# ebiggers/libdeflate

Measured on AMD Instinct MI355X. Metric: compress+decompress MB/s, 64 KiB chunks level 6, higher is better.
Workload: dtype u8

## Files before the change

libdeflate_amd/csrc/deflate_blockend.h:

```cpp

static __device__ u32 block_scan(lds_t *L, u32 v, u32 *total)
{
	const u32 lane = threadIdx.x & 63, wave = threadIdx.x >> 6;
	u32 incl = wave_scan_incl(v);

	if (lane == 63)
		L->scan[0][wave] = incl;
	__syncthreads();
	const u32 sw = lane < NWAVES ? L->scan[0][lane] : 0;
	const u32 iw = wave_scan_incl(sw);
	const u32 base = bcast_lane(iw - sw, wave);
	__syncthreads();
	*total = bcast_lane(iw, NWAVES - 1);
	return base + incl - v;
}

static __device__ u32 block_scan1(lds_t *L, u32 v, u32 *total,
				  u32 *tog)
{
	const u32 lane = threadIdx.x & 63, wave = threadIdx.x >> 6;
	u32 incl = wave_scan_incl(v);
	u32 *sc = L->scan[*tog];

	*tog ^= 1;
// ... 46 lines not shown

static __device__ __forceinline__ u32 *stg_of(lds_t *L)
{
	return (u32 *)L->nxtA;
}

static __device__ __forceinline__ void
stg_put(lds_t *L, const struct outstate *os, u64 bitpos, u64 code,
	u32 nbits)
{
	if (!nbits)
		return;
	u64 rel = bitpos - 8 * os->sg;
	u32 w = (u32)(rel >> 5), s = (u32)rel & 31;
	u32 *stg = stg_of(L);
	u64 lo = code << s;
	atomicOr((u32 *)&stg[w], (u32)lo);
	if (s + nbits > 32)
		atomicOr((u32 *)&stg[w + 1], (u32)(lo >> 32));
	if (s + nbits > 64)
		atomicOr((u32 *)&stg[w + 2], (u32)(code >> (64 - s)));
}

static __device__ __forceinline__ void
stg_flush(lds_t *L, struct outstate *os, bool final)
{
	u32 *stg = stg_of(L);
	u8 *stgb = (u8 *)stg;
	const u32 tid = threadIdx.x;
	u64 done_bytes = final ? (os->bits + 7) / 8 : os->bits / 8;
	u64 rel_end = done_bytes - os->sg;
	s64 first = -(s64)os->sg;
	u32 start = first > 0 ? (u32)first : 0;
	u32 units = final ? (u32)((rel_end + 15) / 16) : (u32)(rel_end / 16);

	__syncthreads();
	for (u32 u = tid; u < units; u += NT) {
		u32 b0 = u * 16, b1 = b0 + 16;
		u8 *g = os->out + (s64)(os->sg + b0);
		if (b0 >= start && b1 <= rel_end) {
			*(uint4 *)g = *(const uint4 *)(stgb + b0);
		} else {
			for (u32 b = b0 < start ? start : b0; b < b1 && b < rel_end; b++)
				g[b - b0] = stgb[b];
		}
	}
	u32 keep_from = units * 16;
	u32 total_words = (u32)((os->bits - 8 * os->sg + 31) / 32) + 1;
	u32 keep_words = final ? 0 : total_words - keep_from / 4;
	u32 v = 0;
	if (tid < keep_words && keep_from / 4 + tid < STG_WORDS + 8)
		v = stg[keep_from / 4 + tid];
	__syncthreads();
	for (u32 i = tid; i < STG_WORDS + 8; i += NT)
		stg[i] = 0;
	if (tid < keep_words)
		stg[tid] = v;
	os->sg += keep_from;
}

static __device__ __forceinline__ void stg_restore(lds_t *L)
{
	u32 *stg = stg_of(L);

	__syncthreads();
	for (u32 i = threadIdx.x; i < STG_WORDS + 8; i += NT)
		stg[i] = i < 6 ? L->carry[i] : 0;
	__syncthreads();
}

static __device__ __forceinline__ void stg_save(lds_t *L, struct outstate *os)
{
	stg_flush(L, os, false);
	if (threadIdx.x < 6)
		L->carry[threadIdx.x] = stg_of(L)[threadIdx.x];
	__syncthreads();
}

static __device__ __forceinline__ void
put_container_header(lds_t *L, struct outstate *os, int format, int level,
		     const u8 *__restrict__ dict_pre, u32 hdr_bytes, u32 tid)
{
	if (tid == 0) {
		if (format == LDA_FMT_BGZF) {
			stg_put(L, os, 0, 0x04088B1Full, 32);
			stg_put(L, os, 32, 0, 32);
			stg_put(L, os, 64, 0xFFu << 8, 16);
			stg_put(L, os, 80, 0x0243420006ull, 48);
		} else if (format == LDA_FMT_GZIP) {
			u32 xfl = level < 2 ? 4 : level >= 8 ? 2 : 0;
			stg_put(L, os, 0, 0x00088B1Full, 32);
			stg_put(L, os, 32, 0, 32);
			stg_put(L, os, 64, xfl | (0xFFu << 8), 16);
		} else {
			u32 fl = level < 2 ? 0 : level < 6 ? 1 :
				 level < 8 ? 2 : 3;
			u32 h = (0x78u << 8) | (fl << 6);
			if (dict_pre) {
				h |= 0x20;
				h += (31 - h % 31) % 31;
				stg_put(L, os, 16, __builtin_bswap32(((const u32 *)dict_pre)[1]), 32);
			} else {
				h |= 31 - (h % 31);
			}
			stg_put(L, os, 0, ((h & 0xFF) << 8) | (h >> 8), 16);
		}
	}
	os->bits = 8 * hdr_bytes;
}

static __device__ __forceinline__ bool
block_emit(lds_t *L, struct outstate *os, const u32 *__restrict__ tokg, u32 nseq,
	   const u8 *__restrict__ inp, u32 bstart, u32 blen, u32 is_final,
	   bool stored_only, u32 ftr_bytes, u32 *tog, u32 tid, u32 lane, u32 wave)
{
	PROF_DECL;
	PROF_START();
	u32 btype = 0;
	if (!stored_only) {
		if (tid == 0)
			L->freq[256]++;
		__syncthreads();
		{
			u32 *keys = L->M;
			u32 *usedv = L->M + 320;
			u16 *sortedO = (u16 *)(L->M + 324);
			if (tid < 2)
				usedv[tid] = 0;
			__syncthreads();
			for (u32 vt = tid; vt < 320; vt += NT) {
				const u32 f = L->freq[vt];
				if (f) {
					if (vt < 288)
						keys[atomicAdd(&usedv[0], 1u)] = (f << 9) | vt;
					else
						keys[288 + atomicAdd(&usedv[1], 1u)] =
							(f << 9) | (vt - 288);
				}
			}
			__syncthreads();
			{
				const u32 m1 = usedv[0], m2 = usedv[1];
				for (u32 i = tid; i < m1 + m2; i += NT) {
					const bool lit = i < m1;
					const u32 lo = lit ? 0 : 288, m = lit ? m1 : m2;
					const u32 key = keys[lit ? i : 288 + i - m1];
					u32 r = 0;
					for (u32 q = 0; q < m; q++)
						r += keys[lo + q] < key;
					if (lit)
						L->sorted[r] = (u16)(key & 511);
					else
						sortedO[r] = (u16)(key & 511);
				}
			}
			__syncthreads();
			PROF_MARK(10);
			if (wave == 0)
				make_code(L->freq, 288, 15, L->lens, L->codes,
					  L->sorted, HUFF_LITLEN(L),
					  usedv[0], true, lane);
			else if (wave == 1)
// ... 141 lines not shown
			u32 xb = tid == 16 ? 2 : tid == 17 ? 3 : tid == 18 ? 7 : 0;
			dyn += L->pre_freq[tid] * (L->pre_lens[tid] + xb);
		}
		u32 dyn_tot, stat_tot;
		(void)block_scan(L, dyn, &dyn_tot);
		(void)block_scan(L, stat, &stat_tot);
		static const u8 perm[19] = { 16, 17, 18, 0, 8, 7, 9, 6, 10,
					     5, 11, 4, 12, 3, 13, 2, 14,
					     1, 15 };
		u32 nexp = 19;
		while (nexp > 4 && L->pre_lens[perm[nexp - 1]] == 0)
			nexp--;
		u32 cost_dyn = 3 + 5 + 5 + 4 + 3 * nexp + dyn_tot;
		u32 cost_stat = 3 + stat_tot;
		u32 pieces = blen ? (blen + 65534) / 65535 : 1;
		u32 pad = (u32)((0 - (os->bits + 3)) & 7);
		u64 cost_stored = 3 + pad + 32 + 8ull * blen +
				  (u64)(pieces - 1) * 40;
		u64 best = cost_stored;
		btype = 0;
		if (cost_stat < best) {
			best = cost_stat;
			btype = 1;
		}
		if (cost_dyn < best) {
			best = cost_dyn;
			btype = 2;
		}
		if ((os->bits + best + 7) / 8 + ftr_bytes > os->avail)
			return false;
		L->vars[V_TMP3] = nexp;
	} else {
		u32 pieces = blen ? (blen + 65534) / 65535 : 1;
		u64 cost = (u64)pieces * 40 + 8ull * blen;
		if ((os->bits + cost + 7) / 8 + ftr_bytes > os->avail)
			return false;
	}

	PROF_MARK(7);
	stg_restore(L);
	if (btype == 0) {
		u32 done = 0;
		do {
			u32 piece = blen - done > 65535 ? 65535 : blen - done;
			u32 fin = (is_final && done + piece == blen) ? 1 : 0;
			u32 pad = (u32)((0 - (os->bits + 3)) & 7);
			if (tid == 0) {
				stg_put(L, os, os->bits, fin, 3);
				u64 b = os->bits + 3 + pad;
				stg_put(L, os, b, piece | ((u64)(piece ^ 0xFFFF) << 16), 32);
			}
			os->bits += 3 + pad + 32;
			__syncthreads();
			for (u32 w0 = 0; w0 < piece; w0 += 2048) {
				u32 cnt = piece - w0 < 2048 ? piece - w0 : 2048;
				stg_flush(L, os, false);
				__syncthreads();
				for (u32 j = tid; j < cnt; j += NT) {
					u32 pos = bstart + done + w0 + j;
					stg_put(L, os, os->bits + 8ull * j, inp[pos], 8);
				}
				os->bits += 8ull * cnt;
				__syncthreads();
			}
			done += piece;
		} while (done < blen);
		stg_flush(L, os, false);
	} else {
		if (btype == 1) {
			__syncthreads();
			for (u32 s = tid; s < 320; s += NT)
				L->lens[s] = s < 144 ? 8 : s < 256 ? 9 :
					     s < 280 ? 7 : s < 288 ? 8 : 5;
			__syncthreads();
			if (tid == 0) {
				u32 nc[16] = { 0 }, bl[16] = { 0 };
				for (u32 s = 0; s < 288; s++)
					bl[L->lens[s]]++;
				u32 code = 0;
				for (u32 d = 1; d < 16; d++) {
					code = (code + bl[d - 1]) << 1;
					nc[d] = code;
				}
				for (u32 s = 0; s < 288; s++) {
					u32 l = L->lens[s];
					L->codes[s] = (u16)(__brev(nc[l]++) >> (32 - l));
				}
				for (u32 s = 0; s < 32; s++)
					L->codes[288 + s] = (u16)(__brev(s) >> 27);
			}
			__syncthreads();
		}
		{
			u64 hcode[VPT];
			u32 hbits[VPT], hsum = 0;
			const u32 nexp = btype == 2 ? L->vars[V_TMP3] : 0;
			const u32 ni = btype == 2 ? L->vars[V_NPRE] : 0;
#pragma unroll
			for (u32 j = 0; j < VPT; j++) {
				const u32 vt = tid * VPT + j;
				hcode[j] = 0;
				hbits[j] = 0;
				if (vt == 0) {
					hcode[j] = is_final | (btype << 1);
					hbits[j] = 3;
					if (btype == 2) {
						u32 nlit = L->vars[V_TMP1], noff = L->vars[V_TMP2];
						hcode[j] |= (u64)((nlit - 257) | ((noff - 1) << 5) |
								  ((nexp - 4) << 10)) << 3;
						hbits[j] = 17;
					}
				} else if (vt <= nexp) {
					static const u8 perm2[19] = { 16, 17, 18, 0, 8, 7,
						9, 6, 10, 5, 11, 4, 12, 3, 13, 2, 14, 1, 15 };
					hcode[j] = L->pre_lens[perm2[vt - 1]];
					hbits[j] = 3;
				} else if (vt <= nexp + ni) {
					u32 it = L->pre_items[vt - nexp - 1];
					u32 sym = it & 31, ex = it >> 5;
					u32 l = L->pre_lens[sym];
					u32 xb = sym == 16 ? 2 : sym == 17 ? 3 :
						 sym == 18 ? 7 : 0;
					hcode[j] = L->pre_codes[sym] | ((u64)ex << l);
					hbits[j] = l + xb;
				}
				hsum += hbits[j];
			}
			u32 htot;
			u32 hoff = block_scan(L, hsum, &htot);
#pragma unroll
			for (u32 j = 0; j < VPT; j++) {
				stg_put(L, os, os->bits + hoff, hcode[j], hbits[j]);
				hoff += hbits[j];
			}
			os->bits += htot;
		}
		stg_flush(L, os, false);

		PROF_MARK(9);
		__builtin_amdgcn_fence(__ATOMIC_ACQUIRE, "workgroup");
		u32 tok_nxt = tid < nseq ? tokg[tid] : 0;
		for (u32 b0 = 0; b0 < nseq; b0 += NT) {
			u64 code = 0;
			u32 nb = 0;
			const u32 tok = tok_nxt;
			if (b0 + NT + tid < nseq)
				tok_nxt = tokg[b0 + NT + tid];
			if (b0 + tid < nseq) {
				if (tok & TOK_MATCH) {
					const u32 len = (tok & 0xFF) + 3, dist = ((tok >> 8) & 0x7FFF) + 1;
					u32 sl, xb, xv, ds, dxb, dxv;
					length_code(len, &sl, &xb, &xv);
					dist_code(dist, &ds, &dxb, &dxv);
					u32 ll = L->lens[257 + sl];
					u32 dl = L->lens[288 + ds];
					u64 v = L->codes[257 + sl];
					u32 sh = ll;
					v |= (u64)xv << sh;
					sh += xb;
					v |= (u64)L->codes[288 + ds] << sh;
					sh += dl;
					v |= (u64)dxv << sh;
					sh += dxb;
					code = v;
					nb = sh;
				} else {
					code = L->codes[tok];
					nb = L->lens[tok];
				}
			}
			u32 tot;
			u32 off = block_scan1(L, nb, &tot, tog);
			stg_put(L, os, os->bits + off, code, nb);
			os->bits += tot;
			if (os->bits - 8 * os->sg + 48 * NT + 64 > 32 * STG_WORDS)
				stg_flush(L, os, false);
		}
		stg_flush(L, os, false);
		__syncthreads();
		if (tid == 0)
			stg_put(L, os, os->bits, L->codes[256], L->lens[256]);
		os->bits += L->lens[256];
		__syncthreads();
	}

	stg_save(L, os);
	PROF_MARK(8);
	return true;
}

static __device__ __forceinline__ void
finish_stream(lds_t *L, struct outstate *os, bool overflow, bool seg_last,
	      int format, u32 ftr_bytes, const u32 *__restrict__ sums, u64 c, u32 n,
	      u64 *__restrict__ out_nbytes, u32 tid)
{
	__syncthreads();
	if (!overflow && !seg_last &&
	    (os->bits + 3 + 7) / 8 + 4 > os->avail)
		overflow = true;
	if (!overflow) {
		stg_restore(L);
		if (!seg_last) {
			u64 fb = 8 * ((os->bits + 3 + 7) / 8);
			if (tid == 0)
				stg_put(L, os, fb, 0xFFFF0000ull, 32);
			os->bits = fb + 32;
			__syncthreads();
		}
		if (ftr_bytes) {
			u32 sum = sums ? sums[c] : 0;
			u64 fb = 8 * ((os->bits + 7) / 8);
			if (tid == 0) {
				if (format != LDA_FMT_ZLIB) {
					stg_put(L, os, fb, sum, 32);
					stg_put(L, os, fb + 32, n, 32);
				} else {
					stg_put(L, os, fb, __builtin_bswap32(sum), 32);
				}
			}
			os->bits = fb + 8 * ftr_bytes;
			__syncthreads();
		}
		stg_flush(L, os, true);
		const u32 size = (u32)((os->bits + 7) / 8);
		if (tid == 0)
			out_nbytes[c] = size;
		if (format == LDA_FMT_BGZF) {
			asm volatile("s_waitcnt vmcnt(0)" ::: "memory");
			__syncthreads();
			if (tid == 0) {
				const u16 bsize = (u16)(size - 1);
// ... 9 lines not shown
```

libdeflate_amd/csrc/deflate_entropy.hip:

```cpp
#include <stddef.h>
#include "device_common.h"
#include "kernels.h"

#define LDA_ENTROPY 1
#define NT LDA_DEFLATE_ENTROPY_THREADS
#define VPT (1024 / NT)
#define NWAVES (NT / 64)
#ifndef ENTROPY_WGS
#define ENTROPY_WGS 4
#endif
static_assert(NT == 256, "ENTROPY_WGS waves per EU are ENTROPY_WGS workgroups per CU");
#define TOK_MATCH 0x80000000u
#define STG_WORDS 1020

struct deflate_lds {
	u32 M[1776];
	u32 freq[320];
	u8 lens[320];
	u16 codes[320];
	u16 sorted[288];
	u32 hw[288];
	u16 pre_items[320 + 8];
	u32 pre_freq[19];
	u8 pre_lens[20];
	u16 pre_codes[20];
	u32 nxtA[STG_WORDS + 8] __attribute__((aligned(16)));
	u32 scan[2][NWAVES + 1];
	u32 carry[6];
	u32 vars[4];
};
static_assert(sizeof(struct deflate_lds) * ENTROPY_WGS <= 163840, "ENTROPY_WGS workgroups per CU");

#ifdef __HIP_DEVICE_COMPILE__
#define AS3 __attribute__((address_space(3)))
#else
#define AS3
#endif
typedef AS3 struct deflate_lds lds_t;

enum { V_TMP1 = 0, V_TMP2, V_TMP3, V_NPRE, V_COUNT };
static_assert(V_COUNT <= sizeof(((struct deflate_lds *)0)->vars) / sizeof(u32), "vars[] holds them all");

#include "deflate_huffman.h"
#include "deflate_blockend.h"

extern "C" __global__ void __launch_bounds__(NT, ENTROPY_WGS)
lda_deflate_entropy_kernel(u64 n_chunks, int format, int level,
			   const u8 *__restrict__ in_base, const u64 *__restrict__ in_offsets,
			   const u64 *__restrict__ in_nbytes, u8 *__restrict__ out_base,
			   const u64 *__restrict__ out_offsets,
			   const u64 *__restrict__ out_avail_arr, u64 *__restrict__ out_nbytes,
			   const u32 *__restrict__ sums, const u32 *__restrict__ seg_info,
			   const u32 *__restrict__ tok_buf, const u32 *__restrict__ blk_buf,
			   u32 tok_stride, u32 blk_stride)
{
	extern __shared__ __attribute__((aligned(16))) u8 lds_raw[];
	lds_t *L = (lds_t *)(uintptr_t)0;
	const u32 tid = threadIdx.x, lane = tid & 63, wave = tid >> 6;
	if ((u32)(uintptr_t)(__attribute__((address_space(3))) u8 *)lds_raw != 0)
		__builtin_trap();
	const u64 c = blockIdx.x;
	if (c >= n_chunks)
		return;
	const u32 nb = blk_buf[c];
	if (nb == LDA_BLK_FUSED)
		return;
	const u32 *__restrict__ desc = blk_buf + LDA_BLK_HDR_WORDS(n_chunks) +
				       c * blk_stride * LDA_BLK_WORDS;
	const u32 *__restrict__ tokg = tok_buf + c * tok_stride;
	const u8 *__restrict__ inp = in_base + in_offsets[c];
	const u32 n = (u32)in_nbytes[c];
	const bool seg_last = seg_info ? seg_info[c] >> 31 : true;
	const u32 hdr_bytes = format == LDA_FMT_GZIP ? 10 : format == LDA_FMT_BGZF ? 18 :
			      format == LDA_FMT_ZLIB ? 2 : 0;
	const u32 ftr_bytes = format == LDA_FMT_GZIP || format == LDA_FMT_BGZF ? 8 :
			      format == LDA_FMT_ZLIB ? 4 : 0;
	bool overflow = nb == LDA_BLK_OVERFLOW;
	struct outstate os;
	os.out = out_base + out_offsets[c];
	os.avail = out_avail_arr[c];
	if (format == LDA_FMT_BGZF && os.avail > LDA_BGZF_MEMBER_MAX)
		os.avail = LDA_BGZF_MEMBER_MAX;
	os.sg = (u64)(0 - ((uintptr_t)os.out & 15));
	os.bits = 0;
	u32 tog = 0;

	for (u32 i = tid; i < STG_WORDS + 8; i += NT)
		stg_of(L)[i] = 0;
	__syncthreads();
	if (!overflow && hdr_bytes)
		put_container_header(L, &os, format, level, NULL, hdr_bytes, tid);
	__syncthreads();
	stg_save(L, &os);

	for (u32 b = 0; b < nb && !overflow; b++) {
		const u32 *__restrict__ d = desc + (size_t)b * LDA_BLK_WORDS;
		for (u32 i = tid; i < 320; i += NT)
			L->freq[i] = d[LDA_BLK_FREQ + i];
		const u32 tok0 = d[LDA_BLK_TOK0], ntok = d[LDA_BLK_NTOK];
		const u32 bstart = d[LDA_BLK_START], bend = d[LDA_BLK_END];
		const u32 flags = d[LDA_BLK_FLAGS];
		__syncthreads();
		if (!block_emit(L, &os, tokg + tok0, ntok, inp, bstart, bend - bstart, flags & 1,
				(flags & LDA_BLK_STORED) != 0, ftr_bytes, &tog, tid, lane, wave))
			overflow = true;
	}
	finish_stream(L, &os, overflow, seg_last, format, ftr_bytes, sums, c, n, out_nbytes, tid);
}

extern "C" size_t lda_deflate_entropy_lds_bytes(void)
{
	return sizeof(struct deflate_lds);
}

// ... 2 lines not shown
```

libdeflate_amd/csrc/device_common.h:

```cpp
#ifndef LDA_DEVICE_COMMON_H
#define LDA_DEVICE_COMMON_H

#include <hip/hip_runtime.h>
#include <stdint.h>

#define LDA_WAVE 64

#ifndef BALLOT_BUILTIN
#define BALLOT_BUILTIN 1
#endif
#if BALLOT_BUILTIN
#define __ballot(p) __builtin_amdgcn_ballot_w64((bool)(p))
#endif

typedef uint8_t u8;
typedef uint16_t u16;
typedef uint32_t u32;
typedef uint64_t u64;
typedef int32_t s32;
typedef int64_t s64;

#define LDA_SUCCESS 0
#define LDA_BAD_DATA 1
#define LDA_SHORT_OUTPUT 2
// ... 58 lines not shown
{
#pragma unroll
	for (int off = 32; off > 0; off >>= 1) {
		u32 lo = __shfl_xor((u32)v, off, 64);
		u32 hi = __shfl_xor((u32)(v >> 32), off, 64);
		v += ((u64)hi << 32) | lo;
	}
	return v;
}

static __device__ __forceinline__ u32 wave_scan_incl(u32 v)
{
	v += __builtin_amdgcn_update_dpp(0, v, 0x111, 0xF, 0xF, true);
	v += __builtin_amdgcn_update_dpp(0, v, 0x112, 0xF, 0xF, true);
	v += __builtin_amdgcn_update_dpp(0, v, 0x114, 0xF, 0xF, true);
	v += __builtin_amdgcn_update_dpp(0, v, 0x118, 0xF, 0xF, true);
	v += __builtin_amdgcn_update_dpp(0, v, 0x142, 0xA, 0xF, false);
	v += __builtin_amdgcn_update_dpp(0, v, 0x143, 0xC, 0xF, false);
	return v;
}

static __device__ __forceinline__ u32 row16_sum(u32 v)
{
	v += __builtin_amdgcn_update_dpp(0, v, 0x111, 0xF, 0xF, true);
	v += __builtin_amdgcn_update_dpp(0, v, 0x112, 0xF, 0xF, true);
	v += __builtin_amdgcn_update_dpp(0, v, 0x114, 0xF, 0xF, true);
	v += __builtin_amdgcn_update_dpp(0, v, 0x118, 0xF, 0xF, true);
	return (u32)__builtin_amdgcn_readlane((int)v, 15);
}

static __device__ __forceinline__ u32 wave_sum(u32 v)
{
	return (u32)__builtin_amdgcn_readlane((int)wave_scan_incl(v), 63);
}

static __device__ __forceinline__ u32 wave_max(u32 v)
{
#pragma unroll
	for (int off = 32; off > 0; off >>= 1) {
		u32 t = __shfl_xor(v, off, 64);
		v = t > v ? t : v;
	}
	return v;
}

static __device__ __forceinline__ void wave_sync(void)
{
	__builtin_amdgcn_fence(__ATOMIC_RELEASE, "wavefront");
	__builtin_amdgcn_wave_barrier();
	__builtin_amdgcn_fence(__ATOMIC_ACQUIRE, "wavefront");
}

#ifdef LDA_PROFILE
#define LDA_PROF_SLOTS 40
static __device__ unsigned long long lda_prof[LDA_PROF_SLOTS];
#define LDA_PROF_DEFINE_READER(name)                                          \
	extern "C" __attribute__((visibility("default"))) void name(           \
		unsigned long long *out)                                      \
	{                                                                     \
		unsigned long long z[LDA_PROF_SLOTS] = { 0 };                 \
		(void)hipDeviceSynchronize();                                 \
		(void)hipMemcpyFromSymbol(out, HIP_SYMBOL(lda_prof), sizeof(z)); \
		(void)hipMemcpyToSymbol(HIP_SYMBOL(lda_prof), z, sizeof(z));  \
	}
#define PROF_DECL unsigned long long prof_t_ = 0
#define PROF_START() do { if (threadIdx.x == 0) prof_t_ = __builtin_readcyclecounter(); } while (0)
#define PROF_MARK(slot) do { if (threadIdx.x == 0) { \
		unsigned long long n_ = __builtin_readcyclecounter(); \
		atomicAdd(&lda_prof[slot], n_ - prof_t_); prof_t_ = n_; } } while (0)
#define PROF_WDECL unsigned long long prof_w_ = 0
#define PROF_W0() do { prof_w_ = __builtin_readcyclecounter(); } while (0)
#define PROF_W(slot) do { unsigned long long n_ = __builtin_readcyclecounter(); \
		if ((threadIdx.x & 63) == 0) atomicAdd(&lda_prof[slot], n_ - prof_w_); \
		prof_w_ = n_; } while (0)
#ifdef LDA_PROFILE_COUNTS
#define PROF_COUNT(slot, v) do { unsigned long long v_ = (v); if (threadIdx.x == 0) \
		atomicAdd(&lda_prof[slot], v_); } while (0)
#define PROF_SEC_DECL unsigned long long sec_[8] = { 0, 0, 0, 0, 0, 0, 0, 0 }, sec_t_ = __builtin_readcyclecounter()
#define PROF_SEC(i) do { unsigned long long n_ = __builtin_readcyclecounter(); \
		sec_[i] += n_ - sec_t_; sec_t_ = n_; } while (0)
#define PROF_SEC_FLUSH(base) do { if (threadIdx.x == 0) for (int i_ = 0; i_ < 4; i_++) \
		atomicAdd(&lda_prof[(base) + i_], sec_[i_]); } while (0)
#define PROF_SEC_FLUSH8(base) do { if (threadIdx.x == 0) for (int i_ = 0; i_ < 8; i_++) \
		atomicAdd(&lda_prof[(base) + i_], sec_[i_]); } while (0)
#define PROF_SEC_ADD(i, v) do { sec_[i] += (v); } while (0)
#else
#define PROF_COUNT(slot, v) do { } while (0)
#define PROF_SEC_DECL
#define PROF_SEC(i) do { } while (0)
#define PROF_SEC_FLUSH(base) do { } while (0)
#define PROF_SEC_FLUSH8(base) do { } while (0)
#define PROF_SEC_ADD(i, v) do { } while (0)
#endif
#else
#define PROF_COUNT(slot, v) do { } while (0)
#define PROF_SEC_DECL
#define PROF_SEC(i) do { } while (0)
#define PROF_SEC_FLUSH(base) do { } while (0)
#define PROF_SEC_FLUSH8(base) do { } while (0)
#define PROF_SEC_ADD(i, v) do { } while (0)
#define PROF_DECL
#define PROF_WDECL
#define PROF_W0() do { } while (0)
#define PROF_W(slot) do { } while (0)
#define PROF_START() do { } while (0)
#define PROF_MARK(slot) do { } while (0)
#define LDA_PROF_DEFINE_READER(name)
// ... 4 lines not shown
```

libdeflate_amd/csrc/host_compress.hip:

```cpp
#include <stdio.h>
#include <stdlib.h>
#include <string.h>
#include <atomic>
#include <new>
#include <algorithm>
#include <vector>

#include "host_objects.h"
#include "kernels.h"

using namespace lda;

struct level_cfg { uint32_t depth, nice, mode; };
static const level_cfg k_levels[13] = {
	{ 0, 0, 0 },
	{ 2, 32, 0 },
	{ 6, 10, 0 },
	{ 12, 14, 0 },
	{ 16, 30, 0 },
	{ 16, 30, 1 },
	{ 35, 65, 1 },
	{ 100, 130, 1 },
	{ 300, 258, 2 },
	{ 600, 258, 2 },
// ... 50 lines not shown
	DeviceGuard on(c->device);
	c->scratch.release();
	c->stage.release();
	c->pinned.release();
	c->meta.release();
	c->bgzf.release();
	c->streams.release();
	free_func_t f = c->free_func;
	c->~libdeflate_compressor();
	f(c);
}

extern "C" LIBDEFLATEAPI size_t
libdeflate_deflate_compress_bound(struct libdeflate_compressor *c, size_t n)
{
	(void)c;
	size_t blocks = (n + 4999) / 5000;
	if (blocks < 1)
		blocks = 1;
	return 5 * blocks + n;
}

extern "C" LIBDEFLATEAPI size_t
libdeflate_zlib_compress_bound(struct libdeflate_compressor *c, size_t n)
{
	return 6 + libdeflate_deflate_compress_bound(c, n);
}

extern "C" LIBDEFLATEAPI size_t
libdeflate_gzip_compress_bound(struct libdeflate_compressor *c, size_t n)
{
	return 18 + libdeflate_deflate_compress_bound(c, n);
}

static size_t dict_window(void)
{
	const size_t tile = lda_deflate_tile();
	return (32768 - 2 * tile - 272) / tile * tile;
}

struct dict_shape { uint32_t tail, pre_len, sinfo; };

static dict_shape shape_dict(int level, size_t dict_nbytes)
{
	const size_t tile = lda_deflate_tile();
	dict_shape d;
	d.tail = level == 0 ? 0 : (uint32_t)std::min(dict_nbytes, dict_window());
	d.pre_len = (uint32_t)((d.tail + tile - 1) / tile * tile);
	d.sinfo = d.pre_len | ((d.pre_len - d.tail) << 16) | 0x80000000u;
	return d;
}

#define LDA_SPLIT_SCRATCH ((size_t)1280 << 20)
#define LDA_SPLIT_MIN_PER_CU 4

struct batch_plan {
	bool small, split;
	size_t grid, per_slice, nslices;
	uint32_t tok_stride, blk_stride;
	size_t cnt_at, sums_at, tok_at, blk_at, dict_at, total;
};

static batch_plan plan_batch(const struct libdeflate_compressor *c, size_t n,
			     size_t max_in, bool seg, bool dict)
{
	batch_plan p = {};
	p.small = max_in <= lda_deflate_small_max() && c->level <= 9 && !seg && !dict &&
		  !env_cfg().no_small;
	const size_t tile = lda_deflate_tile();
	const size_t tok_stride = align_up(max_in, 16);
	const size_t blk_stride = std::max<size_t>(1, (tok_stride + tile - 1) / tile);
	const size_t per_buf = tok_stride * 4 + blk_stride * LDA_BLK_WORDS * 4 + 4;
	const size_t num_cus = (size_t)device_ctx()->num_cus;
	p.split = !p.small && c->level <= 9 && !dict && max_in != SIZE_MAX &&
		  n >= LDA_SPLIT_MIN_PER_CU * num_cus &&
		  per_buf <= LDA_SPLIT_SCRATCH && tok_stride <= 0xFFFFFFF0u;
	p.per_slice = p.split ? std::min(n, LDA_SPLIT_SCRATCH / per_buf) : n;
	p.per_slice = std::max<size_t>(p.per_slice, 1);
	p.nslices = (n + p.per_slice - 1) / p.per_slice;
	const size_t grid_max = num_cus * (p.small ? lda_deflate_small_wgs() : 1);
	p.grid = std::min(p.per_slice, grid_max);
	p.cnt_at = p.grid * lda_deflate_seq_words() * 8;
	p.sums_at = p.cnt_at + align_up(12 * p.nslices, 16);
	p.dict_at = p.tok_at = align_up(p.sums_at + n * 4, 64);
	p.total = p.sums_at + n * 4;
	if (dict)
		p.total = p.dict_at + LDA_DICT_BLK_HDR + dict_window();
	if (p.split) {
		p.tok_stride = (uint32_t)tok_stride;
		p.blk_stride = (uint32_t)blk_stride;
		p.blk_at = align_up(p.tok_at + p.per_slice * tok_stride * 4, 64);
		p.total = p.blk_at + (LDA_BLK_HDR_WORDS(p.per_slice) +
				      p.per_slice * blk_stride * LDA_BLK_WORDS) * 4;
	}
	return p;
}

static int
compress_batch_impl(struct libdeflate_compressor *c, int format, size_t n,
		    const void *d_in, const uint64_t *d_in_offsets,
		    const uint64_t *d_in_nbytes, void *d_out,
		    const uint64_t *d_out_offsets, const uint64_t *d_out_avail,
		    uint64_t *d_out_nbytes, void *stream,
		    const uint32_t *d_seg_info, size_t max_in_nbytes = SIZE_MAX,
		    const void *d_dict = NULL, size_t dict_nbytes = 0)
{
	if (!c) {
		set_error("compress_batch: bad argument");
		return LIBDEFLATE_AMD_BAD_ARG;
	}
	DeviceGuard on(c->device);
	if (!on.ok())
		return LIBDEFLATE_AMD_NO_DEVICE;
	DeviceCtx *ctx = device_ctx();
	hipStream_t st = (hipStream_t)stream;

	if (!ctx)
		return LIBDEFLATE_AMD_NO_DEVICE;
	if (n == 0)
		return LIBDEFLATE_AMD_OK;
	if (!c || !d_in || !d_in_offsets || !d_in_nbytes || !d_out ||
	    !d_out_offsets || !d_out_avail || !d_out_nbytes ||
	    format < LIBDEFLATE_AMD_DEFLATE || format > LIBDEFLATE_AMD_BGZF) {
		set_error("compress_batch: bad argument");
		return LIBDEFLATE_AMD_BAD_ARG;
	}
	const bool dict = d_dict && dict_nbytes;
	const batch_plan pl = plan_batch(c, n, max_in_nbytes, d_seg_info != NULL, dict);
	const bool small = pl.small;
	uint8_t *scr = (uint8_t *)c->scratch.reserve(pl.total);
	if (!scr)
		return LIBDEFLATE_AMD_OOM;
	uint32_t *next_chunk = (uint32_t *)(scr + pl.cnt_at);
	LDA_HIP_TRY(hipMemsetAsync(next_chunk, 0, align_up(12 * pl.nslices, 16), st),
		    LIBDEFLATE_AMD_NO_DEVICE);
	uint8_t *blk = NULL;
	if (dict) {
		const dict_shape sh = shape_dict(c->level, dict_nbytes);
		blk = scr + pl.dict_at;
		hipLaunchKernelGGL(lda_dict_prep_kernel, dim3(1), dim3(256), 0, st,
				   (const uint8_t *)d_dict, (uint64_t)dict_nbytes, sh.tail,
				   sh.pre_len, sh.sinfo, blk);
		LDA_HIP_TRY(hipGetLastError(), LIBDEFLATE_AMD_NO_DEVICE);
		if (format == LIBDEFLATE_AMD_ZLIB) {
			int rc = libdeflate_amd_adler32_batch(1, d_dict, (const uint64_t *)(blk + 16),
							      (const uint64_t *)(blk + 24), NULL,
							      (uint32_t *)(blk + 4), stream);
			if (rc != LIBDEFLATE_AMD_OK)
				return rc;
		}
	}
	uint32_t *sums = NULL;
	if (format != LIBDEFLATE_AMD_DEFLATE) {
		sums = (uint32_t *)(scr + pl.sums_at);
		int rc = format == LIBDEFLATE_AMD_GZIP || format == LIBDEFLATE_AMD_BGZF ?
			libdeflate_amd_crc32_batch(n, d_in, d_in_offsets,
						   d_in_nbytes, NULL, sums, stream) :
			libdeflate_amd_adler32_batch(n, d_in, d_in_offsets,
						     d_in_nbytes, NULL, sums, stream);
		if (rc != LIBDEFLATE_AMD_OK)
			return rc;
	}
	const size_t lds = small ? lda_deflate_small_lds_bytes() : lda_deflate_lds_bytes();
	if (!ctx->deflate_attr_set.load(std::memory_order_acquire)) {
		LDA_HIP_TRY(hipFuncSetAttribute(
				(const void *)lda_deflate_small_kernel,
				hipFuncAttributeMaxDynamicSharedMemorySize,
				(int)lda_deflate_small_lds_bytes()), LIBDEFLATE_AMD_NO_DEVICE);
		LDA_HIP_TRY(hipFuncSetAttribute(
				(const void *)lda_deflate_batch_kernel,
				hipFuncAttributeMaxDynamicSharedMemorySize,
				(int)lda_deflate_lds_bytes()), LIBDEFLATE_AMD_NO_DEVICE);
		LDA_HIP_TRY(hipFuncSetAttribute(
				(const void *)lda_deflate_opt_kernel,
				hipFuncAttributeMaxDynamicSharedMemorySize,
				(int)lda_deflate_lds_bytes()), LIBDEFLATE_AMD_NO_DEVICE);
		LDA_HIP_TRY(hipFuncSetAttribute(
				(const void *)lda_deflate_fused_kernel,
				hipFuncAttributeMaxDynamicSharedMemorySize,
				(int)lda_deflate_lds_bytes()), LIBDEFLATE_AMD_NO_DEVICE);
		ctx->deflate_attr_set.store(true, std::memory_order_release);
	}
	const level_cfg &lv = k_levels[c->level];
	if (!pl.split && (small || lv.mode == 3)) {
		hipLaunchKernelGGL(small ? lda_deflate_small_kernel : lda_deflate_opt_kernel,
				   dim3((unsigned)pl.grid),
				   dim3(small ? LDA_DEFLATE_SMALL_THREADS : LDA_DEFLATE_THREADS),
				   lds, st, (uint64_t)n, format, c->level,
				   lv.depth, lv.nice, lv.mode, (const uint8_t *)d_in,
				   d_in_offsets, d_in_nbytes, (uint8_t *)d_out,
				   d_out_offsets, d_out_avail, d_out_nbytes, sums,
				   (uint64_t *)scr, d_seg_info, next_chunk, (const uint8_t *)blk);
		LDA_HIP_TRY(hipGetLastError(), LIBDEFLATE_AMD_NO_DEVICE);
		return LIBDEFLATE_AMD_OK;
	}
	if (!pl.split) {
		hipLaunchKernelGGL(lda_deflate_fused_kernel, dim3((unsigned)pl.grid),
				   dim3(LDA_DEFLATE_THREADS), lds, st, (uint64_t)n, format,
				   c->level, lv.depth, lv.nice, lv.mode, (const uint8_t *)d_in,
				   d_in_offsets, d_in_nbytes, (uint8_t *)d_out,
				   d_out_offsets, d_out_avail, d_out_nbytes, sums,
				   (uint64_t *)scr, d_seg_info, next_chunk, (const uint8_t *)blk,
				   (const uint32_t *)NULL, (const uint32_t *)NULL);
		LDA_HIP_TRY(hipGetLastError(), LIBDEFLATE_AMD_NO_DEVICE);
		return LIBDEFLATE_AMD_OK;
	}
	uint32_t *tok = (uint32_t *)(scr + pl.tok_at), *bd = (uint32_t *)(scr + pl.blk_at);
	for (size_t k = 0; k < pl.nslices; k++) {
		const size_t lo = k * pl.per_slice, nk = std::min(pl.per_slice, n - lo);
		const uint32_t *sk = sums ? sums + lo : NULL;
		const uint32_t *gk = d_seg_info ? d_seg_info + lo : NULL;
		hipLaunchKernelGGL(lda_deflate_batch_kernel, dim3((unsigned)std::min(nk, pl.grid)),
				   dim3(LDA_DEFLATE_THREADS), lds, st, (uint64_t)nk, format,
				   c->level, lv.depth, lv.nice, lv.mode, (const uint8_t *)d_in,
				   d_in_offsets + lo, d_in_nbytes + lo, (uint8_t *)d_out,
				   d_out_offsets + lo, d_out_avail + lo, d_out_nbytes + lo, sk,
				   (uint64_t *)scr, gk, next_chunk + k, (const uint8_t *)NULL,
				   tok, bd, pl.tok_stride, pl.blk_stride, next_chunk + 2 * pl.nslices + k);
		LDA_HIP_TRY(hipGetLastError(), LIBDEFLATE_AMD_NO_DEVICE);
		hipLaunchKernelGGL(lda_deflate_entropy_kernel, dim3((unsigned)nk),
				   dim3(LDA_DEFLATE_ENTROPY_THREADS), lda_deflate_entropy_lds_bytes(),
				   st, (uint64_t)nk, format, c->level, (const uint8_t *)d_in,
				   d_in_offsets + lo, d_in_nbytes + lo, (uint8_t *)d_out,
				   d_out_offsets + lo, d_out_avail + lo, d_out_nbytes + lo, sk, gk,
				   (const uint32_t *)tok, (const uint32_t *)bd, pl.tok_stride,
				   pl.blk_stride);
		LDA_HIP_TRY(hipGetLastError(), LIBDEFLATE_AMD_NO_DEVICE);
		hipLaunchKernelGGL(lda_deflate_fused_kernel, dim3((unsigned)std::min(nk, pl.grid)),
				   dim3(LDA_DEFLATE_THREADS), lds, st, (uint64_t)nk, format,
				   c->level, lv.depth, lv.nice, lv.mode, (const uint8_t *)d_in,
				   d_in_offsets + lo, d_in_nbytes + lo, (uint8_t *)d_out,
				   d_out_offsets + lo, d_out_avail + lo, d_out_nbytes + lo, sk,
				   (uint64_t *)scr, gk, next_chunk + pl.nslices + k,
				   (const uint8_t *)NULL, (const uint32_t *)bd,
				   (const uint32_t *)(next_chunk + 2 * pl.nslices + k));
		LDA_HIP_TRY(hipGetLastError(), LIBDEFLATE_AMD_NO_DEVICE);
	}
	return LIBDEFLATE_AMD_OK;
}

extern "C" LIBDEFLATEAPI int
libdeflate_amd_compress_batch_dict(struct libdeflate_compressor *c, int format,
				   size_t n, const void *d_dict, size_t dict_nbytes,
				   const void *d_in, const uint64_t *d_in_offsets,
				   const uint64_t *d_in_nbytes, void *d_out,
				   const uint64_t *d_out_offsets,
				   const uint64_t *d_out_avail,
				   uint64_t *d_out_nbytes, void *stream)
{
	if (format != LIBDEFLATE_AMD_DEFLATE && format != LIBDEFLATE_AMD_ZLIB) {
		set_error("compress_batch_dict: format %d takes no dictionary", format);
		return LIBDEFLATE_AMD_BAD_ARG;
	}
	if (dict_nbytes && !d_dict) {
		set_error("compress_batch_dict: bad argument");
		return LIBDEFLATE_AMD_BAD_ARG;
	}
	return compress_batch_impl(c, format, n, d_in, d_in_offsets, d_in_nbytes,
				   d_out, d_out_offsets, d_out_avail,
				   d_out_nbytes, stream, NULL, SIZE_MAX, d_dict, dict_nbytes);
}

extern "C" LIBDEFLATEAPI int
libdeflate_amd_compress_batch(struct libdeflate_compressor *c, int format,
			      size_t n, const void *d_in,
			      const uint64_t *d_in_offsets,
			      const uint64_t *d_in_nbytes, void *d_out,
			      const uint64_t *d_out_offsets,
			      const uint64_t *d_out_avail,
			      uint64_t *d_out_nbytes, void *stream)
{
	return compress_batch_impl(c, format, n, d_in, d_in_offsets, d_in_nbytes,
				   d_out, d_out_offsets, d_out_avail,
				   d_out_nbytes, stream, NULL);
}

extern "C" LIBDEFLATEAPI int
libdeflate_amd_compress_batch_bounded(struct libdeflate_compressor *c, int format,
				      size_t n, const void *d_in,
// ... 447 lines not shown
```

libdeflate_amd/csrc/kernels.h:

```cpp
#ifndef LDA_KERNELS_H
#define LDA_KERNELS_H

#include <hip/hip_runtime.h>
#include <stdint.h>

extern "C" __global__ void
lda_crc32_batch_kernel(uint64_t n_chunks, const uint8_t *base,
		       const uint64_t *offsets, const uint64_t *nbytes,
		       const uint32_t *init, uint32_t *out,
		       const uint32_t *g_tables, const uint32_t *xpow8);
extern "C" __global__ void
lda_adler32_batch_kernel(uint64_t n_chunks, const uint8_t *base,
			 const uint64_t *offsets, const uint64_t *nbytes,
			 const uint32_t *init, uint32_t *out);
#define LDA_DICT_BLK_HDR 64
extern "C" __global__ void
lda_dict_prep_kernel(const uint8_t *dict, uint64_t dict_nbytes, uint32_t tail,
		     uint32_t pre_len, uint32_t sinfo, uint8_t *blk);

extern "C" __global__ void
lda_inflate_batch_kernel(uint64_t n_chunks, int format, uint32_t lpw,
			 const uint8_t *in_base,
			 const uint64_t *in_offsets, const uint64_t *in_nbytes,
			 uint8_t *out_base, const uint64_t *out_offsets,
// ... 16 lines not shown
			 uint32_t *order);
extern "C" size_t lda_inflate_tokcap(void);
extern "C" size_t lda_inflate_window_bytes(void);
extern "C" __global__ void
lda_inflate_finalize_kernel(uint64_t n_chunks, int format, int exact_fill,
			    const uint8_t *in_base, const uint64_t *in_offsets,
			    const uint64_t *out_avail, const uint32_t *sums,
			    int32_t *results, uint64_t *actual_in,
			    uint64_t *actual_out);

#define LDA_DEFLATE_THREADS 1024
#define LDA_BLK_TOK0 0
#define LDA_BLK_NTOK 1
#define LDA_BLK_START 2
#define LDA_BLK_END 3
#define LDA_BLK_FLAGS 4
#define LDA_BLK_STORED 2u
#define LDA_BLK_FREQ 8
#define LDA_BLK_WORDS (LDA_BLK_FREQ + 320)
#define LDA_BLK_OVERFLOW 0xFFFFFFFFu
#define LDA_BLK_FUSED 0xFFFFFFFEu
#define LDA_BLK_LIST(n) (((n) + 15) / 16 * 16)
#define LDA_BLK_HDR_WORDS(n) (2 * LDA_BLK_LIST(n))
extern "C" __global__ void
lda_deflate_batch_kernel(uint64_t n_chunks, int format, int level,
			 uint32_t depth, uint32_t nice, uint32_t mode,
			 const uint8_t *in_base, const uint64_t *in_offsets,
			 const uint64_t *in_nbytes, uint8_t *out_base,
			 const uint64_t *out_offsets, const uint64_t *out_avail,
			 uint64_t *out_nbytes, const uint32_t *sums,
			 uint64_t *seq_scratch, const uint32_t *seg_info,
			 uint32_t *next_chunk, const uint8_t *dict_pre,
			 uint32_t *tok_buf, uint32_t *blk_buf, uint32_t tok_stride,
			 uint32_t blk_stride, uint32_t *fused_cnt);
extern "C" __global__ void
lda_deflate_fused_kernel(uint64_t n_chunks, int format, int level,
			 uint32_t depth, uint32_t nice, uint32_t mode,
			 const uint8_t *in_base, const uint64_t *in_offsets,
			 const uint64_t *in_nbytes, uint8_t *out_base,
			 const uint64_t *out_offsets, const uint64_t *out_avail,
			 uint64_t *out_nbytes, const uint32_t *sums,
			 uint64_t *seq_scratch, const uint32_t *seg_info,
			 uint32_t *next_chunk, const uint8_t *dict_pre,
			 const uint32_t *blk_buf, const uint32_t *fused_cnt);
#define LDA_DEFLATE_ENTROPY_THREADS 256
extern "C" __global__ void
lda_deflate_entropy_kernel(uint64_t n_chunks, int format, int level,
			   const uint8_t *in_base, const uint64_t *in_offsets,
			   const uint64_t *in_nbytes, uint8_t *out_base,
			   const uint64_t *out_offsets, const uint64_t *out_avail,
			   uint64_t *out_nbytes, const uint32_t *sums,
			   const uint32_t *seg_info, const uint32_t *tok_buf,
			   const uint32_t *blk_buf, uint32_t tok_stride,
			   uint32_t blk_stride);
extern "C" size_t lda_deflate_entropy_lds_bytes(void);
extern "C" __global__ void
lda_deflate_opt_kernel(uint64_t n_chunks, int format, int level,
		       uint32_t depth, uint32_t nice, uint32_t mode,
		       const uint8_t *in_base, const uint64_t *in_offsets,
		       const uint64_t *in_nbytes, uint8_t *out_base,
		       const uint64_t *out_offsets, const uint64_t *out_avail,
		       uint64_t *out_nbytes, const uint32_t *sums,
		       uint64_t *seq_scratch, const uint32_t *seg_info,
		       uint32_t *next_chunk, const uint8_t *dict_pre);
#define LDA_DEFLATE_SMALL_THREADS 256
extern "C" __global__ void
lda_deflate_small_kernel(uint64_t n_chunks, int format, int level,
			 uint32_t depth, uint32_t nice, uint32_t mode,
			 const uint8_t *in_base, const uint64_t *in_offsets,
			 const uint64_t *in_nbytes, uint8_t *out_base,
			 const uint64_t *out_offsets, const uint64_t *out_avail,
			 uint64_t *out_nbytes, const uint32_t *sums,
			 uint64_t *seq_scratch, const uint32_t *seg_info,
			 uint32_t *next_chunk, const uint8_t *dict_pre);
extern "C" size_t lda_deflate_small_lds_bytes(void);
extern "C" size_t lda_deflate_small_max(void);
extern "C" size_t lda_deflate_small_wgs(void);
extern "C" size_t lda_deflate_tile(void);
extern "C" size_t lda_deflate_lds_bytes(void);
extern "C" size_t lda_deflate_seq_words(void);

extern "C" size_t lda_inflate_lds_per_stream(void);
extern "C" size_t lda_inflate_lds_shared(void);

#define LDA_SCAN_BLOCK 2048
extern "C" __global__ void
lda_scan_local_kernel(uint64_t n, const uint64_t *sizes, uint64_t *offsets,
		      uint64_t *block_sums);
extern "C" __global__ void
lda_scan_blocks_kernel(uint64_t nblocks, uint64_t *block_sums);
extern "C" __global__ void
lda_compact_copy_kernel(uint64_t n, const uint8_t *in_base,
			const uint64_t *in_offsets, const uint64_t *sizes,
			uint8_t *out_base, uint64_t *offsets,
			const uint64_t *block_sums);
extern "C" __global__ void
lda_bgzf_desc_kernel(uint64_t m, uint64_t n, uint64_t *in_off, uint64_t *in_n,
		     uint64_t *slot_off, uint64_t *slot_avail);
extern "C" __global__ void
lda_bgzf_copy_kernel(uint64_t m, const uint8_t *slots, const uint64_t *sizes,
		     const uint64_t *offsets, const uint64_t *block_sums, uint8_t *out,
		     uint64_t out_avail, uint32_t eof_bytes, uint64_t *index);
extern "C" __global__ void
lda_bgzf_finalize_kernel(uint64_t m, uint64_t n, const uint64_t *sizes,
			 const uint64_t *total_at, uint8_t *out, uint64_t out_avail,
			 uint32_t eof_bytes, uint64_t *out_nbytes, uint64_t *index);

// ... 11 lines not shown
```

Before: 33120.

## Vectorize entropy token encoding, widen staging, direct-copy stored blocks, dynamic chunk queue

Token encoding in the entropy kernel now loads four tokens per thread as a uint4 and looks up precomputed literal, length and offset tables in LDS. Each thread packs its four codes into a 64-bit word accumulator and writes them with one scan and a few stores or atomics, which cuts per-token scans and syncs. The staging buffer is doubled, and the flush only clears the words that were used. Stored blocks copy their aligned middle straight to global memory with 16-byte stores instead of going through staging. Chunks are claimed through an atomic counter instead of blockIdx, which needs extra scratch and changes the LDS footprint and possibly occupancy.

```diff
diff --git a/libdeflate_amd/csrc/deflate_blockend.h b/libdeflate_amd/csrc/deflate_blockend.h
--- a/libdeflate_amd/csrc/deflate_blockend.h
+++ b/libdeflate_amd/csrc/deflate_blockend.h
@@ -122,7 +122,12 @@
 	if (tid < keep_words && keep_from / 4 + tid < STG_WORDS + 8)
 		v = stg[keep_from / 4 + tid];
 	__syncthreads();
-	for (u32 i = tid; i < STG_WORDS + 8; i += NT)
+#if LDA_ENTROPY
+	const u32 clear_words = total_words < STG_WORDS + 8 ? total_words : STG_WORDS + 8;
+#else
+	const u32 clear_words = STG_WORDS + 8;
+#endif
+	for (u32 i = tid; i < clear_words; i += NT)
 		stg[i] = 0;
 	if (tid < keep_words)
 		stg[tid] = v;
@@ -178,6 +183,125 @@
 	}
 	os->bits = 8 * hdr_bytes;
 }
+
+#if LDA_ENTROPY
+#define ENC_K 4
+#define ENC_LIT 0
+#define ENC_LEN 256
+#define ENC_OFF 512
+#define ENC_TAB_WORDS 544
+static_assert(ENC_TAB_WORDS <= sizeof(((struct deflate_lds *)0)->M) / sizeof(u32), "the tables live in M[]");
+static_assert(32 * STG_WORDS >= 48 * ENC_K * NT + 64 + 8 * 16 + 8, "a worst-case window fits the staging area");
+
+static __device__ __forceinline__ void enc_tables_build(lds_t *L, u32 tid)
+{
+	u32 *tab = L->M;
+
+	for (u32 i = tid; i < 256; i += NT) {
+		u32 sl, xb, xv;
+		tab[ENC_LIT + i] = L->codes[i] | ((u32)L->lens[i] << 24);
+		length_code(i + 3, &sl, &xb, &xv);
+		const u32 ll = L->lens[257 + sl];
+		tab[ENC_LEN + i] = L->codes[257 + sl] | (xv << ll) | ((ll + xb) << 24);
+	}
+	if (tid < 30) {
+		const u32 xb = tid < 4 ? 0 : (tid >> 1) - 1;
+		tab[ENC_OFF + tid] = L->codes[288 + tid] | ((u32)L->lens[288 + tid] << 16) | (xb << 20);
+	}
+}
+
+static __device__ __forceinline__ u64 enc_token(const u32 *tab, u32 tok, bool valid, u32 *nbits)
+{
+	const bool match = (tok & TOK_MATCH) != 0;
+	const u32 e = tab[(match ? ENC_LEN : ENC_LIT) + (tok & 0xFF)];
+	const u32 d = (tok >> 8) & 0x7FFF;
+	const u32 hb = 31 - __builtin_clz(d | 2);
+	const u32 slot = d < 4 ? d : 2 * hb + ((d >> (hb - 1)) & 1);
+	const u32 o = tab[ENC_OFF + slot];
+	const u32 n1 = e >> 24, ol = (o >> 16) & 15, oxb = o >> 20;
+	const u32 ov = (o & 0xFFFF) | ((d & ((1u << oxb) - 1)) << ol);
+	u64 v = (e & 0xFFFFFF) | (match ? (u64)ov << n1 : 0);
+	u32 n = n1 + (match ? ol + oxb : 0);
+
+	*nbits = valid ? n : 0;
+	return valid ? v : 0;
+}
+
+template <int J>
+static __device__ __forceinline__ void enc_acc(u64 (&a)[4], u64 v, u32 pos)
+{
+	const u32 q = pos >> 6, sh = pos & 63;
+	const u64 lo = v << sh, hi = (v >> 1) >> (63 - sh);
+
+	if (J == 0) {
+		a[0] = lo;
+		a[1] = hi;
+		a[2] = a[3] = 0;
+	} else {
+		a[0] |= q == 0 ? lo : 0;
+		a[1] |= q == 0 ? hi : q == 1 ? lo : 0;
+		if (J < 3) {
+			a[2] |= q == 1 ? hi : 0;
+		} else {
+			a[2] |= q == 1 ? hi : q == 2 ? lo : 0;
+			a[3] |= q == 2 ? hi : 0;
+		}
+	}
+}
+
+static __device__ __forceinline__ void
+encode_tokens(lds_t *L, struct outstate *os, const u32 *__restrict__ tokg, u32 nseq,
+	      u32 *tog, u32 tid)
+{
+	const u32 *tab = L->M;
+	u32 *stg = stg_of(L);
+	const u32 mis = ((u32)(uintptr_t)tokg >> 2) & (ENC_K - 1);
+	const uint4 *__restrict__ tok4 = (const uint4 *)(tokg - mis);
+	const u32 end = nseq + mis;
+
+	uint4 nxt = make_uint4(0, 0, 0, 0);
+	if (ENC_K * tid < end)
+		nxt = tok4[tid];
+	for (u32 b0 = 0; b0 < end; b0 += ENC_K * NT) {
+		const u32 i0 = b0 + ENC_K * tid;
+		const uint4 t = nxt;
+		if (i0 + ENC_K * NT < end)
+			nxt = tok4[(i0 + ENC_K * NT) / ENC_K];
+		u32 n0, n1, n2, n3;
+		const u64 v0 = enc_token(tab, t.x, i0 >= mis && i0 < end, &n0);
+		const u64 v1 = enc_token(tab, t.y, i0 + 1 >= mis && i0 + 1 < end, &n1);
+		const u64 v2 = enc_token(tab, t.z, i0 + 2 >= mis && i0 + 2 < end, &n2);
+		const u64 v3 = enc_token(tab, t.w, i0 + 3 >= mis && i0 + 3 < end, &n3);
+		const u32 nb = n0 + n1 + n2 + n3;
+		u32 tot;
+		const u32 off = block_scan1(L, nb, &tot, tog);
+		const u32 p = (u32)(os->bits - 8 * os->sg) + off;
+		const u32 w = p >> 5, s = p & 31;
+		u64 a[4];
+		enc_acc<0>(a, v0, s);
+		enc_acc<1>(a, v1, s + n0);
+		enc_acc<2>(a, v2, s + n0 + n1);
+		enc_acc<3>(a, v3, s + n0 + n1 + n2);
+		if (nb) {
+			const u32 last = (s + nb - 1) >> 5;
+			const u32 wd[7] = { (u32)a[0], (u32)(a[0] >> 32), (u32)a[1], (u32)(a[1] >> 32),
+					    (u32)a[2], (u32)(a[2] >> 32), (u32)a[3] };
+			atomicOr(&stg[w], wd[0]);
+#pragma unroll
+			for (u32 i = 1; i < 7; i++) {
+				if (i < last)
+					stg[w + i] = wd[i];
+				else if (i == last)
+					atomicOr(&stg[w + i], wd[i]);
+			}
+		}
+		os->bits += tot;
+		if (os->bits - 8 * os->sg + 48 * ENC_K * NT + 64 > 32 * STG_WORDS)
+			stg_flush(L, os, false);
+	}
+	stg_flush(L, os, false);
+}
+#endif
 
 static __device__ __forceinline__ bool
 block_emit(lds_t *L, struct outstate *os, const u32 *__restrict__ tokg, u32 nseq,
@@ -425,6 +549,34 @@
 			}
 			os->bits += 3 + pad + 32;
 			__syncthreads();
+#if LDA_ENTROPY
+			{
+				const u8 *__restrict__ src = inp + bstart + done;
+				u8 *dst = os->out + (s64)(os->bits / 8);
+				u32 head = (0 - (u32)(uintptr_t)dst) & 15;
+				head = head < piece ? head : piece;
+				const u32 mid = (piece - head) & ~15u;
+				const u32 tail = piece - head - mid;
+				if (tid < head)
+					stg_put(L, os, os->bits + 8 * tid, src[tid], 8);
+				os->bits += 8 * head;
+				stg_flush(L, os, false);
+				for (u32 u = tid; u < mid / 16; u += NT) {
+					uint4 v;
+					__builtin_memcpy(&v, src + head + 16 * u, 16);
+					*(uint4 *)(dst + head + 16 * u) = v;
+				}
+				if (mid) {
+					os->bits += 8ull * mid;
+					os->sg += mid;
+				}
+				__syncthreads();
+				if (tid < tail)
+					stg_put(L, os, os->bits + 8 * tid, src[head + mid + tid], 8);
+				os->bits += 8 * tail;
+				__syncthreads();
+			}
+#else
 			for (u32 w0 = 0; w0 < piece; w0 += 2048) {
 				u32 cnt = piece - w0 < 2048 ? piece - w0 : 2048;
 				stg_flush(L, os, false);
@@ -436,6 +588,7 @@
 				os->bits += 8ull * cnt;
 				__syncthreads();
 			}
+#endif
 			done += piece;
 		} while (done < blen);
 		stg_flush(L, os, false);
@@ -464,6 +617,10 @@
 			}
 			__syncthreads();
 		}
+#if LDA_ENTROPY
+		enc_tables_build(L, tid);
+		PROF_MARK(40);
+#endif
 		{
 			u64 hcode[VPT];
 			u32 hbits[VPT], hsum = 0;
@@ -511,6 +668,10 @@
 		stg_flush(L, os, false);
 
 		PROF_MARK(9);
+#if LDA_ENTROPY
+		__builtin_amdgcn_fence(__ATOMIC_ACQUIRE, "workgroup");
+		encode_tokens(L, os, tokg, nseq, tog, tid);
+#else
 		__builtin_amdgcn_fence(__ATOMIC_ACQUIRE, "workgroup");
 		u32 tok_nxt = tid < nseq ? tokg[tid] : 0;
 		for (u32 b0 = 0; b0 < nseq; b0 += NT) {
@@ -550,6 +711,7 @@
 				stg_flush(L, os, false);
 		}
 		stg_flush(L, os, false);
+#endif
 		__syncthreads();
 		if (tid == 0)
 			stg_put(L, os, os->bits, L->codes[256], L->lens[256]);
diff --git a/libdeflate_amd/csrc/deflate_entropy.hip b/libdeflate_amd/csrc/deflate_entropy.hip
--- a/libdeflate_amd/csrc/deflate_entropy.hip
+++ b/libdeflate_amd/csrc/deflate_entropy.hip
@@ -11,7 +11,7 @@
 #endif
 static_assert(NT == 256, "ENTROPY_WGS waves per EU are ENTROPY_WGS workgroups per CU");
 #define TOK_MATCH 0x80000000u
-#define STG_WORDS 1020
+#define STG_WORDS 2044
 
 struct deflate_lds {
 	u32 M[1776];
@@ -52,14 +52,17 @@
 			   const u64 *__restrict__ out_avail_arr, u64 *__restrict__ out_nbytes,
 			   const u32 *__restrict__ sums, const u32 *__restrict__ seg_info,
 			   const u32 *__restrict__ tok_buf, const u32 *__restrict__ blk_buf,
-			   u32 tok_stride, u32 blk_stride)
+			   u32 tok_stride, u32 blk_stride, u32 *__restrict__ next_chunk)
 {
 	extern __shared__ __attribute__((aligned(16))) u8 lds_raw[];
 	lds_t *L = (lds_t *)(uintptr_t)0;
 	const u32 tid = threadIdx.x, lane = tid & 63, wave = tid >> 6;
 	if ((u32)(uintptr_t)(__attribute__((address_space(3))) u8 *)lds_raw != 0)
 		__builtin_trap();
-	const u64 c = blockIdx.x;
+	if (tid == 0)
+		L->vars[V_TMP1] = atomicAdd(next_chunk, 1u);
+	__syncthreads();
+	const u64 c = (u32)__builtin_amdgcn_readfirstlane((int)L->vars[V_TMP1]);
 	if (c >= n_chunks)
 		return;
 	const u32 nb = blk_buf[c];
diff --git a/libdeflate_amd/csrc/device_common.h b/libdeflate_amd/csrc/device_common.h
--- a/libdeflate_amd/csrc/device_common.h
+++ b/libdeflate_amd/csrc/device_common.h
@@ -134,7 +134,7 @@
 }
 
 #ifdef LDA_PROFILE
-#define LDA_PROF_SLOTS 40
+#define LDA_PROF_SLOTS 48
 static __device__ unsigned long long lda_prof[LDA_PROF_SLOTS];
 #define LDA_PROF_DEFINE_READER(name)                                          \
 	extern "C" __attribute__((visibility("default"))) void name(           \
diff --git a/libdeflate_amd/csrc/host_compress.hip b/libdeflate_amd/csrc/host_compress.hip
--- a/libdeflate_amd/csrc/host_compress.hip
+++ b/libdeflate_amd/csrc/host_compress.hip
@@ -126,7 +126,9 @@
 }
 
 #define LDA_SPLIT_SCRATCH ((size_t)1280 << 20)
+#ifndef LDA_SPLIT_MIN_PER_CU
 #define LDA_SPLIT_MIN_PER_CU 4
+#endif
 
 struct batch_plan {
 	bool small, split;
@@ -155,7 +157,7 @@
 	const size_t grid_max = num_cus * (p.small ? lda_deflate_small_wgs() : 1);
 	p.grid = std::min(p.per_slice, grid_max);
 	p.cnt_at = p.grid * lda_deflate_seq_words() * 8;
-	p.sums_at = p.cnt_at + align_up(12 * p.nslices, 16);
+	p.sums_at = p.cnt_at + 16 * p.nslices;
 	p.dict_at = p.tok_at = align_up(p.sums_at + n * 4, 64);
 	p.total = p.sums_at + n * 4;
 	if (dict)
@@ -206,7 +208,7 @@
 	if (!scr)
 		return LIBDEFLATE_AMD_OOM;
 	uint32_t *next_chunk = (uint32_t *)(scr + pl.cnt_at);
-	LDA_HIP_TRY(hipMemsetAsync(next_chunk, 0, align_up(12 * pl.nslices, 16), st),
+	LDA_HIP_TRY(hipMemsetAsync(next_chunk, 0, 16 * pl.nslices, st),
 		    LIBDEFLATE_AMD_NO_DEVICE);
 	uint8_t *blk = NULL;
 	if (dict) {
@@ -298,7 +300,7 @@
 				   d_in_offsets + lo, d_in_nbytes + lo, (uint8_t *)d_out,
 				   d_out_offsets + lo, d_out_avail + lo, d_out_nbytes + lo, sk, gk,
 				   (const uint32_t *)tok, (const uint32_t *)bd, pl.tok_stride,
-				   pl.blk_stride);
+				   pl.blk_stride, next_chunk + 3 * pl.nslices + k);
 		LDA_HIP_TRY(hipGetLastError(), LIBDEFLATE_AMD_NO_DEVICE);
 		hipLaunchKernelGGL(lda_deflate_fused_kernel, dim3((unsigned)std::min(nk, pl.grid)),
 				   dim3(LDA_DEFLATE_THREADS), lds, st, (uint64_t)nk, format,
diff --git a/libdeflate_amd/csrc/kernels.h b/libdeflate_amd/csrc/kernels.h
--- a/libdeflate_amd/csrc/kernels.h
+++ b/libdeflate_amd/csrc/kernels.h
@@ -92,7 +92,7 @@
 			   uint64_t *out_nbytes, const uint32_t *sums,
 			   const uint32_t *seg_info, const uint32_t *tok_buf,
 			   const uint32_t *blk_buf, uint32_t tok_stride,
-			   uint32_t blk_stride);
+			   uint32_t blk_stride, uint32_t *next_chunk);
 extern "C" size_t lda_deflate_entropy_lds_bytes(void);
 extern "C" __global__ void
 lda_deflate_opt_kernel(uint64_t n_chunks, int format, int level,
```

After: 34580, median of 6. +4.4%, better.
